# RtrMmmt/MPI-BiCGStab

Hardware: NVIDIA H100
Metric: BiCGStab iterations/sec (higher is better)
Workload: dtype f64

## Files before the change

include/bicgstab_b200.h:

```cpp
#ifndef BICGSTAB_B200_H
#define BICGSTAB_B200_H

#include <stddef.h>
#include <stdint.h>

#ifdef __cplusplus
extern "C" {
#endif

#ifndef MATRIX_H

typedef char MM_typecode[4];

typedef struct {
    double       *val;
    unsigned int *col;
    unsigned int *ptr;
    unsigned int  nz, rows, cols;
} CSR_Matrix;

typedef struct {
    unsigned int nz, rows, cols;
    MM_typecode  code;
    int         *recvcounts;
// ... 118 lines not shown
int bicg_spmv(bicg_matrix *m, const double *x_loc, double *y_loc);

int bicg_spmv_time(bicg_matrix *m, int reps, double *ms, double *bytes);

int bicg_profile_solve(bicg_matrix *m, int method, int iters, int krr, int nrr, double class_ms[3], int class_launches[3]);

int bicg_debug_vec_phase(bicg_matrix *m, int phase, const double coef[3], double *vecs, double dots[8]);
int bicg_debug_spmv_epi(bicg_matrix *m, int epi, double *vecs, double dots[8]);
int bicg_debug_get_vec(bicg_matrix *m, int id, double *out);
int bicg_debug_get_scalars(bicg_matrix *m, double out[13]);
int bicg_debug_resident_ctas(bicg_matrix *m);
int bicg_debug_coded_ctas(bicg_matrix *m);
int bicg_debug_stream_codes(bicg_matrix *m, int on);
int bicg_debug_packed_ctas(bicg_matrix *m);
int bicg_debug_stream_values(bicg_matrix *m, int on);

int bicg_last_history(double *out, int cap);
const bicg_stats *bicg_last_stats(void);

void *bicg_stream(void);
int   bicg_device(void);
void  bicg_synchronize(void);
void *bicg_host_alloc(size_t bytes);
void  bicg_host_free(void *p);

void bicg_plan_partition(int n, int world, int *counts, int *displs);
void bicg_plan_partition_nnz(const unsigned int *row_nnz, int n, int world, int *counts, int *displs);
int  bicg_plan_tiles(const unsigned int *ptr, int rows, int rows_per_tile, int cap_nnz, int *tile_row,
                     int tile_row_cap);
int  bicg_plan_cta_tiles(const unsigned int *ptr, int rows, int ctas, int rows_per_tile, const unsigned char *row_extra,
// ... 22 lines not shown
```

mpi-bicgstab_b200/_lib.py:

```python
import ctypes as C
import os

_HERE = os.path.dirname(os.path.abspath(__file__))
LIB_PATH = os.path.join(_HERE, "libbicgstab_b200.so")


class CSR_Matrix(C.Structure):
    _fields_ = [("val", C.POINTER(C.c_double)), ("col", C.POINTER(C.c_uint)), ("ptr", C.POINTER(C.c_uint)),
                ("nz", C.c_uint), ("rows", C.c_uint), ("cols", C.c_uint)]


class INFO_Matrix(C.Structure):
    _fields_ = [("nz", C.c_uint), ("rows", C.c_uint), ("cols", C.c_uint), ("code", C.c_char * 4),
                ("recvcounts", C.POINTER(C.c_int)), ("displs", C.POINTER(C.c_int))]


class bicg_stats(C.Structure):
    _fields_ = [("iters", C.c_int), ("converged", C.c_int), ("final_res", C.c_double), ("loop_ms", C.c_double),
                ("h2d_ms", C.c_double), ("d2h_ms", C.c_double), ("upload_ms", C.c_double),
                ("h2d_bytes", C.c_uint64), ("d2h_bytes", C.c_uint64), ("kernel_launches", C.c_int),
                ("spmv_lanes", C.c_int), ("spmv_kind", C.c_int)]


class bicg_result(C.Structure):
# ... 54 lines not shown
    "bicg_matrix_shift_history": (C.c_int, [C.c_void_p, _P(C.c_double), C.c_int]),
    "bicg_shift_residuals": (C.c_int, [C.c_void_p, C.c_void_p, C.c_void_p, C.c_void_p, C.c_int, C.c_int, _P(C.c_double)]),
    "bicg_last_shift_error": (C.c_int, [_P(C.c_double), C.c_int]),
    "bicg_spmv": (C.c_int, [C.c_void_p, C.c_void_p, C.c_void_p]),
    "bicg_spmv_time": (C.c_int, [C.c_void_p, C.c_int, _P(C.c_double), _P(C.c_double)]),
    "bicg_profile_solve": (C.c_int, [C.c_void_p, C.c_int, C.c_int, C.c_int, C.c_int, _P(C.c_double), _P(C.c_int)]),
    "bicg_debug_vec_phase": (C.c_int, [C.c_void_p, C.c_int, _P(C.c_double), C.c_void_p, _P(C.c_double)]),
    "bicg_debug_spmv_epi": (C.c_int, [C.c_void_p, C.c_int, C.c_void_p, _P(C.c_double)]),
    "bicg_debug_get_vec": (C.c_int, [C.c_void_p, C.c_int, C.c_void_p]),
    "bicg_debug_get_scalars": (C.c_int, [C.c_void_p, _P(C.c_double)]),
    "bicg_debug_resident_ctas": (C.c_int, [C.c_void_p]),
    "bicg_debug_coded_ctas": (C.c_int, [C.c_void_p]),
    "bicg_debug_stream_codes": (C.c_int, [C.c_void_p, C.c_int]),
    "bicg_debug_packed_ctas": (C.c_int, [C.c_void_p]),
    "bicg_debug_stream_values": (C.c_int, [C.c_void_p, C.c_int]),
    "bicg_last_history": (C.c_int, [_P(C.c_double), C.c_int]),
    "bicg_last_stats": (_P(bicg_stats), []),
    "bicg_stream": (C.c_void_p, []),
    "bicg_device": (C.c_int, []),
    "bicg_synchronize": (None, []),
    "bicg_host_alloc": (C.c_void_p, [C.c_size_t]),
    "bicg_host_free": (None, [C.c_void_p]),
    "bicg_plan_partition": (None, [C.c_int, C.c_int, _P(C.c_int), _P(C.c_int)]),
    "bicg_plan_partition_nnz": (None, [_P(C.c_uint), C.c_int, C.c_int, _P(C.c_int), _P(C.c_int)]),
    "bicg_plan_tiles": (C.c_int, [_P(C.c_uint), C.c_int, C.c_int, C.c_int, _P(C.c_int), C.c_int]),
    "bicg_plan_cta_tiles": (C.c_int, [_P(C.c_uint), C.c_int, C.c_int, C.c_int, C.c_void_p, C.c_int, _P(C.c_int), C.c_int,
                                      _P(C.c_int), _P(C.c_uint)]),
    "bicg_plan_cta_tiles_capped": (C.c_int, [_P(C.c_uint), C.c_int, C.c_int, C.c_int, C.c_int, _P(C.c_int), _P(C.c_uint), _P(C.c_int),
                                             C.c_int, _P(C.c_int), _P(C.c_uint)]),
    "bicg_plan_halo_runs": (C.c_int, [_P(CSR_Matrix), _P(INFO_Matrix), C.c_int, C.c_int, C.c_int, _P(C.c_int), C.c_int]),
# ... 26 lines not shown
```

mpi-bicgstab_b200/api.py:

```python
import ctypes as C

import numpy as np

from ._lib import ALLGATHER_FN, CSR_Matrix, INFO_Matrix, bicg_result, bicg_shift_result, bicg_stats, lib

METHODS = {"bicgstab": 0, "ca_bicgstab": 1, "pipe_bicgstab": 2, "pipe_bicgstab_rr": 3}
SHIFTED_METHODS = {"shifted_lopbicg_switching": 0, "shifted_lopbicgstab": 1, "shifted_pipe_lopbicgstab": 2}
SHIFTED_SOLVE_EX = dict(SHIFTED_METHODS, shifted_lopbicg=3)
GEN_KINDS = {"stencil15": 0, "laplace5": 1, "random": 2, "convdiff": 3}


def _dptr(a):
    return a.ctypes.data_as(C.c_void_p)


class MatrixBlock:

    def __init__(self, world):
        self.diag = CSR_Matrix()
        self.offd = CSR_Matrix()
        self.info = INFO_Matrix()
        self._recvcounts = (C.c_int * world)()
        self._displs = (C.c_int * world)()
        self.info.recvcounts = C.cast(self._recvcounts, C.POINTER(C.c_int))
# ... 430 lines not shown
    def resident_ctas(self):
        return int(lib.bicg_debug_resident_ctas(self.h))

    def coded_ctas(self):
        return int(lib.bicg_debug_coded_ctas(self.h))

    def stream_codes(self, on):
        return bool(lib.bicg_debug_stream_codes(self.h, 1 if on else 0))

    def packed_ctas(self):
        return int(lib.bicg_debug_packed_ctas(self.h))

    def stream_values(self, on):
        return bool(lib.bicg_debug_stream_values(self.h, 1 if on else 0))

    def spmv_time(self, reps=20):
        ms, by = C.c_double(), C.c_double()
        lib.bicg_spmv_time(self.h, reps, C.byref(ms), C.byref(by))
        return ms.value, by.value

    def profile(self, method, iters, krr=0, nrr=0):
        ms = (C.c_double * 3)()
        cnt = (C.c_int * 3)()
        rc = lib.bicg_profile_solve(self.h, METHODS[method], iters, int(krr), int(nrr), ms, cnt)
        if rc != 0:
            raise RuntimeError("bicg_profile_solve failed")
        return list(ms), list(cnt)

    def destroy(self):
        if self.h:
# ... 47 lines not shown
```

mpi-bicgstab_b200/csrc/engine.hpp:

```cpp
#pragma once
#include "bicgstab_b200.h"
#include "dev.cuh"
#include "plan.hpp"
#include "spmv.cuh"
#include "vec.cuh"
#include "mega.cuh"

#include <cstdio>
#include <cstdlib>
#include <functional>
#include <initializer_list>
#include <map>
#include <string>
#include <vector>

namespace bicg {

[[noreturn]] void fatal(const char *fmt, ...);
#define BICG_CUDA(call)                                                                              \
    do {                                                                                             \
        cudaError_t e_ = (call);                                                                     \
        if (e_ != cudaSuccess)                                                                       \
            ::bicg::fatal("bicgstab_b200: CUDA error %s at %s:%d: %s", cudaGetErrorName(e_), __FILE__, \
                          __LINE__, cudaGetErrorString(e_));                                          \
// ... 87 lines not shown
void load_config_from_env(Config &c);
int  set_option(Config &c, const char *key, const char *value);


struct SpmvPlan {
    int kind = 0, lanes = 1, threads = 256, stages = 3, cap = 0, grid = 0, ctas_per_sm = 1;
    size_t smem = 0;
    int ntiles = 0;
    int *d_tile_row = nullptr;
    unsigned *d_tile_nz = nullptr;
    double ms = 0.0;
};

struct MegaPlan {
    bool ok = false;
    int threads = 512, lanes = 1, stages = 2, cap = 0, grid = 0;
    size_t smem = 0;
    size_t res_smem = 0;
    int ntiles = 0;
    int *d_tile_row = nullptr;
    unsigned *d_tile_nz = nullptr;
    int *d_cta_tile = nullptr;
    int4 *d_cta_dep = nullptr;
    unsigned short *d_col16 = nullptr;
    bool stream_codes = true;
    ValTable *d_vtab = nullptr;
    unsigned char *d_vhi = nullptr;
    unsigned short *d_vmid = nullptr;
    unsigned *d_vlo = nullptr;
    bool stream_values = true;
    int *d_tile_flag = nullptr;
// ... 155 lines not shown
```

mpi-bicgstab_b200/csrc/matrix.cu:

```cuda
#include "engine.hpp"

#include <algorithm>
#include <climits>
#include <cmath>
#include <cstdarg>
#include <cstring>
#include <ctime>
#include <thread>

namespace bicg {

void fatal(const char *fmt, ...)
{
    va_list ap;
    va_start(ap, fmt);
    vfprintf(stderr, fmt, ap);
    va_end(ap);
    fputc('\n', stderr);
    exit(1);
}

namespace {

enum class Parse { Int, Double, Spmv };
// ... 442 lines not shown
    if (m->n_loc < 1) return;
    const int G = std::min(c.sm_count, MEGA_MAX_CTAS);
    const long long SMEM_MAX = 222 * 1024;
    const int lanes = c.cfg.mega_lanes > 0 ? c.cfg.mega_lanes : mega_lanes_for(m->mean_row);
    if (lanes != 1 && c.cfg.mega != 2 && c.cfg.mega_lanes == 0) return;
    for (int threads : {512, 256}) {
        if (c.cfg.mega_threads && c.cfg.mega_threads != threads) continue;
        if (!mega_has_variant(threads, lanes)) continue;
        const int rpt = threads / lanes;
        std::vector<int> tile_row, cta_tile, tile_flag;
        std::vector<unsigned> tile_nz;
        const int cap_limit = (int)(((SMEM_MAX / 2 - (long long)(rpt + 8) * 4) / 12) / 32 * 32) - 64;
        const unsigned max_tile_nnz = plan_cta_tiles(h_ptr, m->n_loc, G, rpt, row_extra.empty() ? nullptr : row_extra.data(),
                                                     c.cfg.boundary_weight, tile_row, cta_tile, cap_limit, &tile_nz, &tile_flag, c.cfg.row_weight);
        const int cap = round_up((long long)max_tile_nnz + 30, 32);
        const long long stage = (long long)cap * 12 + (long long)(rpt + 8) * 4;
        int stages = (int)std::min<long long>(4, SMEM_MAX / stage);
        if (stages < 2) continue;
        bool chunked = false;
        for (int f : tile_flag) chunked = chunked || f != 0;
        mp.chunked = chunked;
        mp.threads = threads; mp.lanes = lanes; mp.stages = stages; mp.cap = cap; mp.grid = G;
        mp.smem = mega_smem_bytes(cap, stages, threads, lanes);
        mp.res_smem = 0;
        if (lanes == 1 && !chunked) {
            size_t need = 0;
            for (int g = 0; g < G; ++g) {
                const int r0 = tile_row[(size_t)cta_tile[(size_t)g]], r1 = tile_row[(size_t)cta_tile[(size_t)g + 1]];
                need = std::max(need, mega_resident_bytes(h_ptr[r1] - h_ptr[r0], r1 - r0));
            }
            if (need <= (size_t)SMEM_MAX) mp.res_smem = std::max<size_t>(need, 16);
        }
        mp.ntiles = (int)tile_row.size() - 1;
        mp.cta_row.assign((size_t)G + 1, m->n_loc);
        for (int g = 0; g <= G; ++g) mp.cta_row[(size_t)g] = tile_row[(size_t)cta_tile[(size_t)g]];
        mp.d_tile_row = (decltype(mp.d_tile_row))c.dev_alloc(tile_row.size() * sizeof(int));
        mp.d_tile_nz = (decltype(mp.d_tile_nz))c.dev_alloc(tile_nz.size() * sizeof(unsigned));
        mp.d_cta_tile = (decltype(mp.d_cta_tile))c.dev_alloc(cta_tile.size() * sizeof(int));
// ... 2 lines not shown
        if (chunked) {
            mp.d_tile_flag = (int *)c.dev_alloc(tile_flag.size() * sizeof(int));
            BICG_CUDA(cudaMemcpy(mp.d_tile_flag, tile_flag.data(), tile_flag.size() * sizeof(int), cudaMemcpyHostToDevice));
        }
        BICG_CUDA(cudaMemcpy(mp.d_tile_row, tile_row.data(), tile_row.size() * sizeof(int), cudaMemcpyHostToDevice));
        BICG_CUDA(cudaMemcpy(mp.d_tile_nz, tile_nz.data(), tile_nz.size() * sizeof(unsigned), cudaMemcpyHostToDevice));
        BICG_CUDA(cudaMemcpy(mp.d_cta_tile, cta_tile.data(), cta_tile.size() * sizeof(int), cudaMemcpyHostToDevice));
        launch_mega_dep(m->d_col, m->d_ptr, mp.d_tile_row, mp.d_cta_tile, G, m->ghost_off, mp.d_cta_dep, c.stream);
        BICG_CUDA(cudaGetLastError());
        const size_t pad = 16;
        mp.d_col16 = (unsigned short *)c.dev_alloc((m->nnz + pad) * sizeof(unsigned short));
        BICG_CUDA(cudaMemsetAsync(mp.d_col16 + m->nnz, 0, pad * sizeof(unsigned short), c.stream));
        launch_mega_code(m->d_col, m->d_ptr, mp.d_tile_row, mp.d_cta_tile, G, m->ghost_off, mp.d_cta_dep, mp.d_col16, c.stream);
        BICG_CUDA(cudaGetLastError());
        mp.d_vtab = nullptr; mp.d_vhi = nullptr; mp.d_vmid = nullptr; mp.d_vlo = nullptr;
        if (m->mean_row >= PACK_MIN_MEAN_ROW) {
            mp.d_vtab = (ValTable *)c.dev_alloc((size_t)G * sizeof(ValTable));
            mp.d_vhi = (unsigned char *)c.dev_alloc(m->nnz + pad);
            mp.d_vmid = (unsigned short *)c.dev_alloc((m->nnz + pad) * sizeof(unsigned short));
            mp.d_vlo = (unsigned *)c.dev_alloc((m->nnz + pad) * sizeof(unsigned));
            BICG_CUDA(cudaMemsetAsync(mp.d_vhi + m->nnz, 0, pad, c.stream));
            BICG_CUDA(cudaMemsetAsync(mp.d_vmid + m->nnz, 0, pad * sizeof(unsigned short), c.stream));
            BICG_CUDA(cudaMemsetAsync(mp.d_vlo + m->nnz, 0, pad * sizeof(unsigned), c.stream));
            launch_mega_values(m->d_val, m->d_ptr, mp.d_tile_row, mp.d_cta_tile, G, m->ghost_off, mp.d_cta_dep, mp.d_vtab, mp.d_vhi,
                               mp.d_vmid, mp.d_vlo, c.stream);
            BICG_CUDA(cudaGetLastError());
        }
        mp.ok = true;
        if (c.cfg.verbose)
            fprintf(stderr, "[bicg mega r%d] threads=%d lanes=%d stages=%d cap=%d tiles=%d smem=%zu resident_smem=%zu\n", m->rank, threads, lanes,
                    stages, cap, mp.ntiles, mp.smem, mp.res_smem);
        return;
    }
}

__global__ void __launch_bounds__(256) merge_rows_kernel(int n_loc, const unsigned *__restrict__ dptr, const unsigned *__restrict__ optr,
                                                         const double *__restrict__ dval, const unsigned *__restrict__ dcol,
                                                         const double *__restrict__ oval, const unsigned *__restrict__ ocol,
                                                         const int *__restrict__ runs , int nruns, int ghost_off,
                                                         double *__restrict__ mval, unsigned *__restrict__ mcol)
{
    for (int i = blockIdx.x * blockDim.x + threadIdx.x; i < n_loc; i += gridDim.x * blockDim.x) {
        const unsigned d0 = dptr[i], d1 = dptr[i + 1], o0 = optr[i], o1 = optr[i + 1];
        unsigned k = d0 + o0;
        for (unsigned j = d0; j < d1; ++j, ++k) { mval[k] = dval[j]; mcol[k] = dcol[j]; }
        for (unsigned j = o0; j < o1; ++j, ++k) {
// ... 357 lines not shown
```

mpi-bicgstab_b200/csrc/mega.cu:

```cuda
#include "mega.cuh"
#include "vec_body.cuh"

namespace bicg {

namespace {

constexpr int RED_THREADS = MEGA_MAX_CTAS;
constexpr int RED_WARPS = RED_THREADS / 32;
struct StageHdr { int row0, row1; unsigned a0; int rowa; unsigned lo, hi; int flag; int pad_; };

__device__ __forceinline__ unsigned long long l2_evict_first_policy()
{
    unsigned long long pol;
    asm volatile("createpolicy.fractional.L2::evict_first.b64 %0, 1.0;" : "=l"(pol));
    return pol;
}
__device__ __forceinline__ void tma_load_1d_hint(unsigned dst_smem, const void *src, unsigned bytes, unsigned bar,
                                                 unsigned long long pol)
{
    asm volatile("cp.async.bulk.shared::cluster.global.mbarrier::complete_tx::bytes.L2::cache_hint [%0], [%1], %2, [%3], %4;"
                 ::"r"(dst_smem), "l"(src), "r"(bytes), "r"(bar), "l"(pol) : "memory");
}
__device__ __forceinline__ void poll_pause(unsigned spins)
{
// ... 83 lines not shown
}
__device__ __forceinline__ unsigned val_adj(const ValTable &t, int i)
{
    return i < t.n ? ((unsigned)t.field[i] << 20) - ((unsigned)i << 20) : 0u;
}
__device__ __forceinline__ unsigned lds_u32(unsigned p) { unsigned v; asm volatile("ld.shared.u32 %0, [%1];" : "=r"(v) : "r"(p)); return v; }
__device__ __forceinline__ unsigned lds_u16(unsigned p) { unsigned v; asm volatile("ld.shared.u16 %0, [%1];" : "=r"(v) : "r"(p)); return v; }
__device__ __forceinline__ unsigned lds_u8(unsigned p) { unsigned v; asm volatile("ld.shared.u8 %0, [%1];" : "=r"(v) : "r"(p)); return v; }
struct PackedVal {
    unsigned hm, lo, adj;
    __device__ __forceinline__ operator double() const
    {
        return __hiloint2double((int)(hm + lds_u32(adj + (hm >> 20) * 4u)), (int)lo);
    }
};
__device__ __forceinline__ PackedVal val_load(unsigned adj, unsigned st, unsigned cap, unsigned idx)
{
    const unsigned lo = lds_u32(st + idx * 4u), mid = lds_u16(st + cap * 4u + idx * 2u), hi = lds_u8(st + cap * 6u + idx);
    return PackedVal{(hi << 16) | mid, lo, adj};
}

template <int CT, int LANES>
struct Mega {
    static constexpr int RPT = CT / LANES, PROW = RPT + PROW_PAD, NCW = CT / 32, UNR = (LANES == 1) ? 16 : 8;
    static_assert(CT >= RED_THREADS, "the slot reduction uses one thread per CTA slot");

    const MegaArgs &a;
    MegaShared &sh;
    unsigned char *dyn;
    int tid, lane, my_tiles, row_lo, row_hi;
    unsigned vis;
    unsigned gen;
    unsigned red_epoch;
    unsigned posted_gen;
    unsigned long long halo_epoch;
    int dep_lo, dep_hi;
    unsigned push_slots;
    int ghost_lo, ghost_hi;
    int gs_lo, gs_hi;
    bool reads_ghost;
    bool is_reducer;
    size_t stage_bytes;
    int trace_it, trace_who;
    bool resident;
    bool coded;
    bool packed;
    ResidentPlan rp;
    const double *rs_val; const unsigned short *rs_col; const unsigned *rs_ptr;

    __device__ Mega(const MegaArgs &args, MegaShared &s) : a(args), sh(s) {}

    __device__ bool stop_now() const { return sh.sc.done != 0 || sh.sc.error != 0; }
    __device__ void fail() { sh.flags[3] = 1; }
    __device__ __forceinline__ bool timed_out(unsigned long long t0, unsigned spins) const
    {
        return (spins & 255u) == 0u && globaltimer_ns() - t0 > a.comm.timeout_ns;
    }
// ... 261 lines not shown
                }
#pragma unroll
                for (int u = 0; u < U; ++u) {
                    const double v = rs_val[min(min(j + (unsigned)u, e - 1u), last)];
                    if (j + (unsigned)u < e) acc = fma(v, xv[u], acc);
                }
                j += (unsigned)U;
            }
            row_done<EPI>(row, acc, e0, e1, e2, e3, y, dot);
        }
    }

    template <int EPI, bool CODED, bool PACKED>
    __device__ void spmv_impl(const double *x, double *y, double (&dot)[4])
    {
        const int stages = a.stages, cap = a.cap;
        const int sub = tid % LANES, row_in_tile = tid / LANES;
        const ColWindow w = rp.w;
        double carry = 0.0;
        for (int lt = 0; lt < my_tiles; ++lt, ++vis) {
            const int s = (int)(vis % (unsigned)stages);
            mbar_wait(smem_u32(&sh.full_bar[s]), (vis / (unsigned)stages) & 1u);
            const unsigned char *st = dyn + (size_t)s * stage_bytes;
            const double   *sval = reinterpret_cast<const double *>(st);
            const unsigned *scol = reinterpret_cast<const unsigned *>(sval + cap);
            const unsigned short *scode = reinterpret_cast<const unsigned short *>(scol);
            const unsigned *sptr = scol + cap;
            const unsigned sts = PACKED ? smem_u32(st) : 0u, adj = PACKED ? smem_u32(sh.vadj) : 0u;
            auto column = [&](unsigned idx) { return CODED ? col_decode(w, scode[idx]) : scol[idx]; };
            auto value = [&](unsigned idx) {
                if constexpr (PACKED) return val_load(adj, sts, (unsigned)cap, idx);
                else return sval[idx];
            };
            const StageHdr h = sh.hdr[s];
            if (h.flag != 0) {
                double part[1] = {0.0};
                for (unsigned jj = h.lo + (unsigned)tid; jj < h.hi; jj += 4u * CT) {
                    double pv[4], px[4];
#pragma unroll
                    for (int u = 0; u < 4; ++u) {
                        const unsigned idx = min(jj + (unsigned)(u * CT), h.hi - 1u);
                        pv[u] = (double)value(idx); px[u] = ld_coherent(x + column(idx));
                    }
#pragma unroll
                    for (int u = 0; u < 4; ++u)
                        if (jj + (unsigned)(u * CT) < h.hi) part[0] = fma(pv[u], px[u], part[0]);
// ... 278 lines not shown
            spmv<EPI_NONE>(a.v.w, a.v.t, d4);
            complete<5>(FIN_CAPIPE_END, true);
            if (stop_now()) break;
        }
    }
};

template <int CT, int LANES>
__global__ void __launch_bounds__(CT + 32, 1) bicg_mega_kernel(const __grid_constant__ MegaArgs a)
{
    using M = Mega<CT, LANES>;
    extern __shared__ __align__(128) unsigned char dyn_smem[];
    __shared__ __align__(16) MegaShared sh;

    const int tid = threadIdx.x;
    const int stages = a.stages, cap = a.cap;
    if (tid == 0) {
        for (int s = 0; s < stages; ++s) {
            mbar_init(smem_u32(&sh.full_bar[s]), 1u);
            mbar_init(smem_u32(&sh.empty_bar[s]), (unsigned)M::NCW);
        }
        sh.flags[0] = sh.flags[1] = sh.flags[2] = sh.flags[3] = 0;
        mbar_fence_init();
    }
    __syncthreads();

    const int t0 = a.cta_tile[blockIdx.x], t1 = a.cta_tile[blockIdx.x + 1];
    const int my_tiles = t1 - t0;
    const size_t stage_bytes = (size_t)cap * 12 + (size_t)M::PROW * 4;

    if (tid >= CT) {
        const ResidentPlan rp = tid == CT ? resident_plan(a, t0, t1, LANES) : ResidentPlan{};
        if (tid == CT && my_tiles > 0 && !rp.on) {
            volatile int *flags = sh.flags;
            const unsigned long long pol = l2_evict_first_policy();
            const bool coded = streams_codes(a, rp, my_tiles);
            const bool packed = streams_values(a, coded);
            const unsigned al = packed ? 15u : (coded ? 7u : 3u), cbytes = coded ? 2u : 4u, vbytes = packed ? 7u : 8u;
            const void *cols = coded ? (const void *)a.col16 : (const void *)a.col;
            unsigned v = 0;
            bool stop = false;
            for (;; ++v) {
                const int s = (int)(v % (unsigned)stages);
                if (v >= (unsigned)stages) {
                    const unsigned par = (v / (unsigned)stages - 1u) & 1u;
                    while (!mbar_try_wait(smem_u32(&sh.empty_bar[s]), par)) {
                        if (flags[1]) { stop = true; break; }
                    }
                }
                if (stop || flags[1]) break;
                const int t = t0 + (int)(v % (unsigned)my_tiles);
                const int row0 = a.tile_row[t], row1 = a.tile_row[t + 1];
                const unsigned p0 = a.tile_nz[t], p1 = a.tile_nz[t + 1];
                const auto [a0, cnt, rowa, cntp] = tile_window(row0, row1, p0, p1, al);
                unsigned char *st = dyn_smem + (size_t)s * stage_bytes;
                double   *sval = reinterpret_cast<double *>(st);
                unsigned *scol = reinterpret_cast<unsigned *>(sval + cap);
                unsigned *sptr = scol + cap;
                sh.hdr[s] = StageHdr{row0, row1, a0, rowa, p0 - a0, p1 - a0, a.tile_flag ? a.tile_flag[t] : 0, 0};
                const unsigned bar = smem_u32(&sh.full_bar[s]);
                mbar_arrive_expect_tx(bar, cnt * (vbytes + cbytes) + (unsigned)cntp * 4u);
                if (cnt) {
                    const void *csrc = (const char *)cols + (size_t)a0 * cbytes;
                    if (packed) {
                        tma_load_1d_hint(smem_u32(st), a.vlo + a0, cnt * 4u, bar, pol);
                        tma_load_1d_hint(smem_u32(st + (size_t)cap * 4u), a.vmid + a0, cnt * 2u, bar, pol);
                        tma_load_1d_hint(smem_u32(st + (size_t)cap * 6u), a.vhi + a0, cnt, bar, pol);
                    } else {
                        tma_load_1d_hint(smem_u32(sval), a.val + a0, cnt * 8u, bar, pol);
                    }
                    tma_load_1d_hint(smem_u32(scol), csrc, cnt * cbytes, bar, pol);
                }
                tma_load_1d(smem_u32(sptr), a.ptr + rowa, (unsigned)cntp * 4u, bar);
            }
            const unsigned consumed = (unsigned)flags[2];
            for (unsigned w = consumed; w < v; ++w)
                mbar_wait(smem_u32(&sh.full_bar[w % (unsigned)stages]), (w / (unsigned)stages) & 1u);
        }
    } else {
        M m(a, sh);
        m.dyn = dyn_smem; m.tid = tid; m.lane = tid & 31; m.my_tiles = my_tiles; m.vis = 0u; m.stage_bytes = stage_bytes;
        m.row_lo = a.tile_row[t0]; m.row_hi = a.tile_row[t1];
        m.trace_it = 0;
        m.trace_who = blockIdx.x == 0 ? 0 : (blockIdx.x == gridDim.x / 2 ? 1 : -1);
        m.gen = a.sync->st.gen; m.red_epoch = a.sync->st.red_epoch; m.halo_epoch = a.sync->st.halo_epoch;
        m.posted_gen = m.gen;
        if (tid == 0) sh.sc = *a.sc;

        const int4 dep = a.cta_dep[blockIdx.x];
        const int G = (int)gridDim.x;
        auto cta_of_row = [&](int r) {
            int lo = 0, hi = G;
            while (lo < hi) { const int mid = (lo + hi) >> 1; if (a.tile_row[a.cta_tile[mid]] <= r) lo = mid + 1; else hi = mid; }
            return lo - 1;
        };
        m.dep_lo = 1; m.dep_hi = 0;
// ... 25 lines not shown
        if (m.resident) {
            const size_t nnzp = ((size_t)m.rp.nnz + 7u) & ~(size_t)7u;
            double *sv = reinterpret_cast<double *>(dyn_smem);
            unsigned short *sc16 = reinterpret_cast<unsigned short *>(sv + nnzp);
            unsigned *sp = reinterpret_cast<unsigned *>(sc16 + nnzp);
            for (unsigned i = (unsigned)tid; i < m.rp.nnz; i += (unsigned)CT) {
                sv[i] = a.val[m.rp.nz_lo + i];
                sc16[i] = a.col16[m.rp.nz_lo + i];
            }
            for (int r = tid; r <= m.rp.rows; r += CT) sp[r] = a.ptr[m.rp.row_lo + r] - m.rp.nz_lo;
            m.rs_val = sv; m.rs_col = sc16; m.rs_ptr = sp;
            if (tid == 0) atomicAdd(&a.sync->st.resident_ctas, 1);
        }
        if (m.coded && tid == 0) atomicAdd(&a.sync->st.coded_ctas, 1);
        if (m.packed && tid == 0) atomicAdd(&a.sync->st.packed_ctas, 1);
        nbar(1, CT);
        if (a.comm.world > 1 && (m.reads_ghost || m.gs_hi > m.gs_lo)) {
            if (tid < 32 && !halo_wait_epoch(a.comm, sh.sc.halo_epoch) && tid == 0) { sh.sc.error = 1; sh.sc.done = 1; }
            if (tid < 32) fence_sys();
            nbar(1, CT);
        }
        if (!m.stop_now()) {
            if (a.method == 0) { if (a.comm.world > 1) m.run_bicgstab_multi(); else m.run_bicgstab(); }
            else if (a.method == 1) m.run_ca();
            else m.run_pipe(a.method == 3);
        }
        nbar(1, CT);
        if (tid == 0) {
            sh.flags[2] = (int)m.vis; __threadfence_block(); sh.flags[1] = 1;
            if (blockIdx.x == 0) {
// ... 30 lines not shown
                                                        const int *__restrict__ tile_row, const int *__restrict__ cta_tile,
                                                        int ghost_off, const int4 *__restrict__ dep, unsigned short *__restrict__ col16)
{
    const ColWindow w = col_window(dep[blockIdx.x], ghost_off);
    if (!w.ok) return;
    const int r0 = tile_row[cta_tile[blockIdx.x]], r1 = tile_row[cta_tile[blockIdx.x + 1]];
    if (r1 <= r0) return;
    const unsigned e0 = ptr[r0], e1 = ptr[r1];
    for (unsigned j = e0 + threadIdx.x; j < e1; j += blockDim.x) col16[j] = col_encode(w, ghost_off, col[j]);
}

__global__ void __launch_bounds__(256) mega_value_kernel(const double *__restrict__ val, const unsigned *__restrict__ ptr,
                                                         const int *__restrict__ tile_row, const int *__restrict__ cta_tile,
                                                         int ghost_off, const int4 *__restrict__ dep, ValTable *__restrict__ vtab,
                                                         unsigned char *__restrict__ vhi, unsigned short *__restrict__ vmid,
                                                         unsigned *__restrict__ vlo)
{
    constexpr int W = 4096 / 32;
    __shared__ unsigned seen[W];
    __shared__ int below[W];
    __shared__ int total;
    for (int i = threadIdx.x; i < W; i += blockDim.x) seen[i] = 0u;
    __syncthreads();
    const int r0 = tile_row[cta_tile[blockIdx.x]], r1 = tile_row[cta_tile[blockIdx.x + 1]];
    const unsigned e0 = r1 > r0 ? ptr[r0] : 0u, e1 = r1 > r0 ? ptr[r1] : 0u;
    for (unsigned j = e0 + threadIdx.x; j < e1; j += blockDim.x) {
        const unsigned f = (unsigned)((unsigned long long)__double_as_longlong(val[j]) >> 52), b = 1u << (f & 31u);
        if (!(seen[f >> 5] & b)) atomicOr(&seen[f >> 5], b);
    }
    __syncthreads();
    if (threadIdx.x == 0) {
        int n = 0;
        for (int i = 0; i < W; ++i) { below[i] = n; n += __popc(seen[i]); }
        total = n;
        ValTable t;
        t.n = n <= VAL_TABLE_MAX ? n : 0;
        for (int k = 0; k < VAL_TABLE_MAX; ++k) t.field[k] = 0;
        int k = 0;
        for (int i = 0; i < W && t.n > 0; ++i)
            for (unsigned b = seen[i]; b; b &= b - 1u) t.field[k++] = (unsigned short)(i * 32 + __ffs((int)b) - 1);
        vtab[blockIdx.x] = t;
    }
    __syncthreads();
    if (total == 0 || total > VAL_TABLE_MAX || !col_window(dep[blockIdx.x], ghost_off).ok) return;
    for (unsigned j = e0 + threadIdx.x; j < e1; j += blockDim.x) {
        const unsigned long long bits = (unsigned long long)__double_as_longlong(val[j]);
        const unsigned f = (unsigned)(bits >> 52);
        const unsigned idx = (unsigned)below[f >> 5] + __popc(seen[f >> 5] & ((1u << (f & 31u)) - 1u));
        vhi[j] = (unsigned char)((idx << 4) | ((unsigned)(bits >> 48) & 15u));
        vmid[j] = (unsigned short)(bits >> 32);
        vlo[j] = (unsigned)bits;
    }
}

template <int CT, int LANES>
cudaError_t launch(const MegaArgs &a, int grid, size_t smem, cudaStream_t st)
{
    void *params[1] = {(void *)&a};
    return cudaLaunchCooperativeKernel((const void *)bicg_mega_kernel<CT, LANES>, dim3(grid), dim3(CT + 32), params, smem, st);
}
template <int CT, int LANES>
cudaError_t set_attr()
{
    cudaFuncAttributes fa;
    cudaError_t e = cudaFuncGetAttributes(&fa, bicg_mega_kernel<CT, LANES>);
    if (e != cudaSuccess) return e;
    return cudaFuncSetAttribute(bicg_mega_kernel<CT, LANES>, cudaFuncAttributeMaxDynamicSharedMemorySize,
                                227 * 1024 - (int)fa.sharedSizeBytes);
}

}

size_t mega_smem_bytes(int cap, int stages, int threads, int lanes)
{
    return (size_t)stages * ((size_t)cap * 12u + (size_t)(threads / lanes + PROW_PAD) * 4u);
}

bool mega_has_variant(int threads, int lanes)
{
    if (threads == 256) return lanes == 1;
    return threads == 512 && (lanes == 1 || lanes == 4 || lanes == 8 || lanes == 32);
}

int mega_setup_attributes()
{
    cudaError_t e;
    if ((e = set_attr<256, 1>()) != cudaSuccess) return (int)e;
    if ((e = set_attr<512, 1>()) != cudaSuccess) return (int)e;
    if ((e = set_attr<512, 4>()) != cudaSuccess) return (int)e;
    if ((e = set_attr<512, 8>()) != cudaSuccess) return (int)e;
// ... 16 lines not shown

void launch_mega_dep(const unsigned *col, const unsigned *ptr, const int *tile_row, const int *cta_tile, int grid,
                     int ghost_off, int4 *dep, cudaStream_t st)
{
    mega_dep_kernel<<<grid, 256, 0, st>>>(col, ptr, tile_row, cta_tile, ghost_off, dep);
}

void launch_mega_code(const unsigned *col, const unsigned *ptr, const int *tile_row, const int *cta_tile, int grid,
                      int ghost_off, const int4 *dep, unsigned short *col16, cudaStream_t st)
{
    mega_code_kernel<<<grid, 256, 0, st>>>(col, ptr, tile_row, cta_tile, ghost_off, dep, col16);
}

void launch_mega_values(const double *val, const unsigned *ptr, const int *tile_row, const int *cta_tile, int grid,
                        int ghost_off, const int4 *dep, ValTable *vtab, unsigned char *vhi, unsigned short *vmid,
                        unsigned *vlo, cudaStream_t st)
{
    mega_value_kernel<<<grid, 256, 0, st>>>(val, ptr, tile_row, cta_tile, ghost_off, dep, vtab, vhi, vmid, vlo);
}

}
```

mpi-bicgstab_b200/csrc/mega.cuh:

```cuda
#pragma once
#include "dev.cuh"
#include "vec.cuh"

namespace bicg {

constexpr int MEGA_MAX_CTAS   = 160;
constexpr int MEGA_RING       = 8;
constexpr int MEGA_SLOT_WORDS = 16;

struct alignas(128) MegaSlot { unsigned long long w[MEGA_SLOT_WORDS]; };

struct alignas(128) MegaState {
    unsigned gen;
    unsigned red_epoch;
    unsigned long long halo_epoch;
    int plan_ok[MAX_RANKS];
    int resident_ctas;
    int coded_ctas;
    int packed_ctas;
};

struct MegaSync {
    MegaState st;
    MegaSlot  slot[MEGA_RING][MEGA_MAX_CTAS];
    MegaSlot  mail[2][MAX_RANKS];
};

struct PushPlan {
    int npeers;
    int peer[MAX_RANKS - 1];
    const PushRun *runs[MAX_RANKS - 1];
    int nruns[MAX_RANKS - 1];
    unsigned long long *ll_dst[MAX_RANKS - 1];
    long long ll_stride[MAX_RANKS - 1];
};

enum LLRegion : int { LL_S0 = 0, LL_S1, LL_R, LL_P, LL_Z, LL_X, LL_W, LL_REGIONS };

constexpr int VAL_TABLE_MAX = 16;
struct ValTable { int n; unsigned short field[VAL_TABLE_MAX]; };

constexpr int MEGA_TRACE_ITERS = 256, MEGA_TRACE_SLOTS = 16;

struct MegaArgs {
    Scalars *sc;
    double  *hist;
    CommDev  comm;
    MegaSync *sync;
    MegaSlot *peer_mail[MAX_RANKS];
    int n_ghost;
    const int4 *cta_dep;
    const double   *val;
    const unsigned *col;
    const unsigned short *col16;
    const ValTable *vtab;
    const unsigned char  *vhi;
    const unsigned short *vmid;
    const unsigned       *vlo;
    const unsigned *ptr;
    const int      *tile_row;
    const unsigned *tile_nz;
    const int      *cta_tile;
    const int      *tile_flag;
    int cap, stages;
    int ghost_off;
    int resident;
    int stream_codes;
    int stream_values;
    int smem_bytes;
    double *vec_base; long long vstride;
    VecPtrs v;
    PushPlan push;
    const unsigned long long *ll;
    long long ll_stride;
    int method;
    int krr, nrr;
    unsigned long long *snap;
    int snap_iter;
    unsigned long long *trace;
};

int    launch_mega(int threads, int lanes, int grid, size_t smem, const MegaArgs &a, cudaStream_t st);
int    mega_setup_attributes();
bool   mega_has_variant(int threads, int lanes);
size_t mega_smem_bytes(int cap, int stages, int threads, int lanes);
__host__ __device__ inline size_t mega_resident_bytes(unsigned nnz, int rows)
{
    const size_t nnzp = ((size_t)nnz + 7u) & ~(size_t)7u;
    return nnzp * 10u + ((size_t)rows + 1u) * 4u;
}
void   launch_mega_dep(const unsigned *col, const unsigned *ptr, const int *tile_row, const int *cta_tile, int grid,
                       int ghost_off, int4 *dep, cudaStream_t st);
void   launch_mega_code(const unsigned *col, const unsigned *ptr, const int *tile_row, const int *cta_tile, int grid,
                        int ghost_off, const int4 *dep, unsigned short *col16, cudaStream_t st);
void   launch_mega_values(const double *val, const unsigned *ptr, const int *tile_row, const int *cta_tile, int grid,
                          int ghost_off, const int4 *dep, ValTable *vtab, unsigned char *vhi, unsigned short *vmid,
                          unsigned *vlo, cudaStream_t st);

}
```

mpi-bicgstab_b200/csrc/solve.cu:

```cuda
#include "engine.hpp"
#include "vec_body.cuh"

#include <algorithm>
#include <cmath>
#include <cstring>

namespace bicg {

namespace {

__global__ void reset_state_kernel(Scalars *s, double tol, int max_iter)
{
    s->rTr = s->rTr_old = s->rTs = s->rTy = s->yTy = s->rTw = s->wTw = s->rTz = 0.0;
    s->dot_r = s->dot_zero = 0.0;
    s->alpha = s->beta = s->omega = 0.0;
    s->tol2 = tol * tol;
    for (int k = 0; k < MAX_DOTS; ++k) s->pend[k] = 0.0;
    s->k = 0; s->max_iter = max_iter; s->done = 0; s->converged = 0; s->error = 0; s->ticket = 0u;
}

__global__ void fill_kernel(double *p, int n, double v)
{
    for (int i = blockIdx.x * blockDim.x + threadIdx.x; i < n; i += gridDim.x * blockDim.x) p[i] = v;
}
// ... 203 lines not shown
struct Seq : PhaseLauncher {
    using PhaseLauncher::PhaseLauncher;

    bool mega(int method, int krr, int nrr)
    {
        MegaArgs a{};
        a.sc = m->d_sc; a.hist = m->d_hist; a.comm = m->comm; a.sync = m->d_msync;
        for (int p = 0; p < MAX_RANKS; ++p) a.peer_mail[p] = &m->peer_msync[p]->mail[0][0];
        a.n_ghost = m->n_ghost; a.cta_dep = m->mega.d_cta_dep;
        a.val = m->d_val; a.col = m->d_col; a.col16 = m->mega.d_col16; a.ptr = m->d_ptr;
        a.stream_codes = m->mega.stream_codes ? 1 : 0;
        a.vtab = m->mega.d_vtab; a.vhi = m->mega.d_vhi; a.vmid = m->mega.d_vmid; a.vlo = m->mega.d_vlo;
        a.stream_values = m->mega.stream_values ? 1 : 0;
        a.tile_row = m->mega.d_tile_row; a.tile_nz = m->mega.d_tile_nz; a.cta_tile = m->mega.d_cta_tile;
        a.tile_flag = m->mega.d_tile_flag;
        a.cap = m->mega.cap; a.stages = m->mega.stages;
        a.ghost_off = m->ghost_off;
        size_t smem = m->mega.smem;
        a.resident = (c.cfg.resident && m->mega.res_smem) ? 1 : 0;
        if (a.resident) smem = std::max(smem, m->mega.res_smem);
        a.smem_bytes = (int)smem;
        a.vec_base = m->vec_base; a.vstride = m->vstride;
        a.v = ptrs();
        a.push.npeers = m->world > 1 ? m->npush : 0;
        for (int s = 0; s < a.push.npeers; ++s) {
            const int d = m->push_peer[s];
            a.push.peer[s] = d;
            a.push.runs[s] = m->d_push_runs[s];
            a.push.nruns[s] = m->push_nruns[s];
            a.push.ll_dst[s] = m->peer_ll[d];
            a.push.ll_stride[s] = m->peer_ll_stride[d];
        }
        a.ll = m->d_ll; a.ll_stride = m->ll_stride;
        a.method = method; a.krr = krr; a.nrr = nrr;
        a.trace = m->d_trace;
        a.snap = m->d_trace ? m->d_trace + (size_t)2 * MEGA_TRACE_ITERS * MEGA_TRACE_SLOTS : nullptr;
        a.snap_iter = 50;
        BICG_CUDA(cudaMemsetAsync(&m->d_msync->st.resident_ctas, 0, sizeof(int), stream));
        BICG_CUDA(cudaMemsetAsync(&m->d_msync->st.coded_ctas, 0, sizeof(int), stream));
        BICG_CUDA(cudaMemsetAsync(&m->d_msync->st.packed_ctas, 0, sizeof(int), stream));
        int rc = launch_mega(m->mega.threads, m->mega.lanes, m->mega.grid, smem, a, stream);
        if (rc) {
            (void)cudaGetLastError();
            if (m->world > 1) fatal("bicgstab_b200: rank %d could not launch the persistent kernel: %s", m->rank,
                                    cudaGetErrorString((cudaError_t)rc));
            if (c.cfg.verbose) fprintf(stderr, "[bicg] persistent kernel not launched (%s); using the per-phase kernels\n",
                                       cudaGetErrorString((cudaError_t)rc));
            m->mega.ok = false;
            return false;
        }
        ++launches; ++c.launches;
        return true;
    }

    void bicgstab_init()
// ... 547 lines not shown
    return was;
}

extern "C" int bicg_debug_packed_ctas(bicg_matrix *m)
{
    using namespace bicg;
    Context &c = ctx();
    c.ensure();
    wait_handle(m);
    int n = 0;
    BICG_CUDA(cudaMemcpyAsync(&n, &m->d_msync->st.packed_ctas, sizeof(int), cudaMemcpyDeviceToHost, c.stream));
    BICG_CUDA(cudaStreamSynchronize(c.stream));
    return n;
}

extern "C" int bicg_debug_stream_values(bicg_matrix *m, int on)
{
    const int was = m->mega.stream_values ? 1 : 0;
    m->mega.stream_values = on != 0;
    return was;
}

extern "C" int bicg_profile_solve(bicg_matrix *m, int method, int iters, int krr, int nrr, double class_ms[3], int class_launches[3])
{
    using namespace bicg;
    Context &c = ctx();
    c.ensure();
    Config saved = c.cfg;
    c.cfg.tol = 0.0; c.cfg.max_iter = iters; c.cfg.quiet = 1;
    if (iters + 2 > m->hist_cap) { c.cfg = saved; return -1; }
// ... 16 lines not shown
```

Baseline: 3752.

## Size TMA staging ring per stream format so compact tiles get more stages

Replaces the fixed stage count and fixed 12-byte-per-entry stage layout with a per-format layout (packed 9, coded 10, col32 12 bytes per entry). The producer and consumers now derive the number of ring stages at runtime from the shared-memory budget and the format each CTA streams. The goal is deeper prefetch for compact formats, or a smaller shared-memory footprint when every CTA packs values. It adds a setup-time count of packing CTAs with a host sync, plus a debug counter for the stages actually used; the larger shared allocation could lower occupancy or change residency.

```diff
diff --git a/include/bicgstab_b200.h b/include/bicgstab_b200.h
--- a/include/bicgstab_b200.h
+++ b/include/bicgstab_b200.h
@@ -156,6 +156,7 @@
 int bicg_debug_stream_codes(bicg_matrix *m, int on);
 int bicg_debug_packed_ctas(bicg_matrix *m);
 int bicg_debug_stream_values(bicg_matrix *m, int on);
+int bicg_debug_ring_stages(bicg_matrix *m);
 
 int bicg_last_history(double *out, int cap);
 const bicg_stats *bicg_last_stats(void);
diff --git a/mpi-bicgstab_b200/_lib.py b/mpi-bicgstab_b200/_lib.py
--- a/mpi-bicgstab_b200/_lib.py
+++ b/mpi-bicgstab_b200/_lib.py
@@ -92,6 +92,7 @@
     "bicg_debug_stream_codes": (C.c_int, [C.c_void_p, C.c_int]),
     "bicg_debug_packed_ctas": (C.c_int, [C.c_void_p]),
     "bicg_debug_stream_values": (C.c_int, [C.c_void_p, C.c_int]),
+    "bicg_debug_ring_stages": (C.c_int, [C.c_void_p]),
     "bicg_last_history": (C.c_int, [_P(C.c_double), C.c_int]),
     "bicg_last_stats": (_P(bicg_stats), []),
     "bicg_stream": (C.c_void_p, []),
diff --git a/mpi-bicgstab_b200/api.py b/mpi-bicgstab_b200/api.py
--- a/mpi-bicgstab_b200/api.py
+++ b/mpi-bicgstab_b200/api.py
@@ -468,6 +468,9 @@
     def stream_values(self, on):
         return bool(lib.bicg_debug_stream_values(self.h, 1 if on else 0))
 
+    def ring_stages(self):
+        return int(lib.bicg_debug_ring_stages(self.h))
+
     def spmv_time(self, reps=20):
         ms, by = C.c_double(), C.c_double()
         lib.bicg_spmv_time(self.h, reps, C.byref(ms), C.byref(by))
diff --git a/mpi-bicgstab_b200/csrc/engine.hpp b/mpi-bicgstab_b200/csrc/engine.hpp
--- a/mpi-bicgstab_b200/csrc/engine.hpp
+++ b/mpi-bicgstab_b200/csrc/engine.hpp
@@ -125,7 +125,7 @@
 
 struct MegaPlan {
     bool ok = false;
-    int threads = 512, lanes = 1, stages = 2, cap = 0, grid = 0;
+    int threads = 512, lanes = 1, cap = 0, grid = 0;
     size_t smem = 0;
     size_t res_smem = 0;
     int ntiles = 0;
diff --git a/mpi-bicgstab_b200/csrc/matrix.cu b/mpi-bicgstab_b200/csrc/matrix.cu
--- a/mpi-bicgstab_b200/csrc/matrix.cu
+++ b/mpi-bicgstab_b200/csrc/matrix.cu
@@ -480,14 +480,11 @@
         const unsigned max_tile_nnz = plan_cta_tiles(h_ptr, m->n_loc, G, rpt, row_extra.empty() ? nullptr : row_extra.data(),
                                                      c.cfg.boundary_weight, tile_row, cta_tile, cap_limit, &tile_nz, &tile_flag, c.cfg.row_weight);
         const int cap = round_up((long long)max_tile_nnz + 30, 32);
-        const long long stage = (long long)cap * 12 + (long long)(rpt + 8) * 4;
-        int stages = (int)std::min<long long>(4, SMEM_MAX / stage);
-        if (stages < 2) continue;
+        if (ring_stages(SMEM_MAX, stage_layout(FMT_COL32, cap, rpt + PROW_PAD).bytes) < 2) continue;
         bool chunked = false;
         for (int f : tile_flag) chunked = chunked || f != 0;
         mp.chunked = chunked;
-        mp.threads = threads; mp.lanes = lanes; mp.stages = stages; mp.cap = cap; mp.grid = G;
-        mp.smem = mega_smem_bytes(cap, stages, threads, lanes);
+        mp.threads = threads; mp.lanes = lanes; mp.cap = cap; mp.grid = G;
         mp.res_smem = 0;
         if (lanes == 1 && !chunked) {
             size_t need = 0;
@@ -520,7 +517,10 @@
         launch_mega_code(m->d_col, m->d_ptr, mp.d_tile_row, mp.d_cta_tile, G, m->ghost_off, mp.d_cta_dep, mp.d_col16, c.stream);
         BICG_CUDA(cudaGetLastError());
         mp.d_vtab = nullptr; mp.d_vhi = nullptr; mp.d_vmid = nullptr; mp.d_vlo = nullptr;
+        int packing = 0;
         if (m->mean_row >= PACK_MIN_MEAN_ROW) {
+            int *d_packing = (int *)c.dev_alloc(sizeof(int));
+            BICG_CUDA(cudaMemsetAsync(d_packing, 0, sizeof(int), c.stream));
             mp.d_vtab = (ValTable *)c.dev_alloc((size_t)G * sizeof(ValTable));
             mp.d_vhi = (unsigned char *)c.dev_alloc(m->nnz + pad);
             mp.d_vmid = (unsigned short *)c.dev_alloc((m->nnz + pad) * sizeof(unsigned short));
@@ -529,13 +529,20 @@
             BICG_CUDA(cudaMemsetAsync(mp.d_vmid + m->nnz, 0, pad * sizeof(unsigned short), c.stream));
             BICG_CUDA(cudaMemsetAsync(mp.d_vlo + m->nnz, 0, pad * sizeof(unsigned), c.stream));
             launch_mega_values(m->d_val, m->d_ptr, mp.d_tile_row, mp.d_cta_tile, G, m->ghost_off, mp.d_cta_dep, mp.d_vtab, mp.d_vhi,
-                               mp.d_vmid, mp.d_vlo, c.stream);
+                               mp.d_vmid, mp.d_vlo, d_packing, c.stream);
             BICG_CUDA(cudaGetLastError());
-        }
+            BICG_CUDA(cudaMemcpyAsync(&packing, d_packing, sizeof(int), cudaMemcpyDeviceToHost, c.stream));
+            BICG_CUDA(cudaStreamSynchronize(c.stream));
+            c.dev_free(d_packing);
+        }
+        mp.smem = mega_smem_bytes(cap, threads, lanes, packing == G, SMEM_MAX);
+        int stages[3];
+        for (int fmt = FMT_PACKED; fmt <= FMT_COL32; ++fmt) stages[fmt] = ring_stages(mp.smem, stage_layout(fmt, cap, rpt + PROW_PAD).bytes);
         mp.ok = true;
         if (c.cfg.verbose)
-            fprintf(stderr, "[bicg mega r%d] threads=%d lanes=%d stages=%d cap=%d tiles=%d smem=%zu resident_smem=%zu\n", m->rank, threads, lanes,
-                    stages, cap, mp.ntiles, mp.smem, mp.res_smem);
+            fprintf(stderr, "[bicg mega r%d] threads=%d lanes=%d stages(9/10/12 B per entry)=%d/%d/%d cap=%d tiles=%d smem=%zu "
+                    "resident_smem=%zu\n", m->rank, threads, lanes, packing ? stages[FMT_PACKED] : 0, stages[FMT_CODED], stages[FMT_COL32],
+                    cap, mp.ntiles, mp.smem, mp.res_smem);
         return;
     }
 }
diff --git a/mpi-bicgstab_b200/csrc/mega.cu b/mpi-bicgstab_b200/csrc/mega.cu
--- a/mpi-bicgstab_b200/csrc/mega.cu
+++ b/mpi-bicgstab_b200/csrc/mega.cu
@@ -121,10 +121,14 @@
         return __hiloint2double((int)(hm + lds_u32(adj + (hm >> 20) * 4u)), (int)lo);
     }
 };
-__device__ __forceinline__ PackedVal val_load(unsigned adj, unsigned st, unsigned cap, unsigned idx)
-{
-    const unsigned lo = lds_u32(st + idx * 4u), mid = lds_u16(st + cap * 4u + idx * 2u), hi = lds_u8(st + cap * 6u + idx);
+__device__ __forceinline__ PackedVal val_load(unsigned adj, unsigned plo, unsigned pmid, unsigned phi, unsigned idx)
+{
+    const unsigned lo = lds_u32(plo + idx * 4u), mid = lds_u16(pmid + idx * 2u), hi = lds_u8(phi + idx);
     return PackedVal{(hi << 16) | mid, lo, adj};
+}
+__device__ __forceinline__ int stage_format(bool coded, bool packed)
+{
+    return packed ? FMT_PACKED : (coded ? FMT_CODED : FMT_COL32);
 }
 
 template <int CT, int LANES>
@@ -147,7 +151,6 @@
     int gs_lo, gs_hi;
     bool reads_ghost;
     bool is_reducer;
-    size_t stage_bytes;
     int trace_it, trace_who;
     bool resident;
     bool coded;
@@ -439,22 +442,23 @@
     template <int EPI, bool CODED, bool PACKED>
     __device__ void spmv_impl(const double *x, double *y, double (&dot)[4])
     {
-        const int stages = a.stages, cap = a.cap;
         const int sub = tid % LANES, row_in_tile = tid / LANES;
         const ColWindow w = rp.w;
+        const StageLayout lay = stage_layout(stage_format(CODED, PACKED), a.cap, PROW);
+        const int stages = ring_stages((size_t)a.smem_bytes, lay.bytes);
         double carry = 0.0;
         for (int lt = 0; lt < my_tiles; ++lt, ++vis) {
             const int s = (int)(vis % (unsigned)stages);
             mbar_wait(smem_u32(&sh.full_bar[s]), (vis / (unsigned)stages) & 1u);
-            const unsigned char *st = dyn + (size_t)s * stage_bytes;
+            const unsigned char *st = dyn + (size_t)s * lay.bytes;
             const double   *sval = reinterpret_cast<const double *>(st);
-            const unsigned *scol = reinterpret_cast<const unsigned *>(sval + cap);
+            const unsigned *scol = reinterpret_cast<const unsigned *>(st + lay.col);
+            const unsigned *sptr = reinterpret_cast<const unsigned *>(st + lay.ptr);
+            const unsigned sts = PACKED ? smem_u32(st) : 0u, adj = PACKED ? smem_u32(sh.vadj) : 0u;
             const unsigned short *scode = reinterpret_cast<const unsigned short *>(scol);
-            const unsigned *sptr = scol + cap;
-            const unsigned sts = PACKED ? smem_u32(st) : 0u, adj = PACKED ? smem_u32(sh.vadj) : 0u;
             auto column = [&](unsigned idx) { return CODED ? col_decode(w, scode[idx]) : scol[idx]; };
             auto value = [&](unsigned idx) {
-                if constexpr (PACKED) return val_load(adj, sts, (unsigned)cap, idx);
+                if constexpr (PACKED) return val_load(adj, sts, sts + lay.mid, sts + lay.hi, idx);
                 else return sval[idx];
             };
             const StageHdr h = sh.hdr[s];
@@ -763,9 +767,8 @@
     __shared__ __align__(16) MegaShared sh;
 
     const int tid = threadIdx.x;
-    const int stages = a.stages, cap = a.cap;
     if (tid == 0) {
-        for (int s = 0; s < stages; ++s) {
+        for (int s = 0; s < MEGA_MAX_STAGES; ++s) {
             mbar_init(smem_u32(&sh.full_bar[s]), 1u);
             mbar_init(smem_u32(&sh.empty_bar[s]), (unsigned)M::NCW);
         }
@@ -776,7 +779,6 @@
 
     const int t0 = a.cta_tile[blockIdx.x], t1 = a.cta_tile[blockIdx.x + 1];
     const int my_tiles = t1 - t0;
-    const size_t stage_bytes = (size_t)cap * 12 + (size_t)M::PROW * 4;
 
     if (tid >= CT) {
         const ResidentPlan rp = tid == CT ? resident_plan(a, t0, t1, LANES) : ResidentPlan{};
@@ -785,6 +787,8 @@
             const unsigned long long pol = l2_evict_first_policy();
             const bool coded = streams_codes(a, rp, my_tiles);
             const bool packed = streams_values(a, coded);
+            const StageLayout lay = stage_layout(stage_format(coded, packed), a.cap, M::PROW);
+            const int stages = ring_stages((size_t)a.smem_bytes, lay.bytes);
             const unsigned al = packed ? 15u : (coded ? 7u : 3u), cbytes = coded ? 2u : 4u, vbytes = packed ? 7u : 8u;
             const void *cols = coded ? (const void *)a.col16 : (const void *)a.col;
             unsigned v = 0;
@@ -802,10 +806,7 @@
                 const int row0 = a.tile_row[t], row1 = a.tile_row[t + 1];
                 const unsigned p0 = a.tile_nz[t], p1 = a.tile_nz[t + 1];
                 const auto [a0, cnt, rowa, cntp] = tile_window(row0, row1, p0, p1, al);
-                unsigned char *st = dyn_smem + (size_t)s * stage_bytes;
-                double   *sval = reinterpret_cast<double *>(st);
-                unsigned *scol = reinterpret_cast<unsigned *>(sval + cap);
-                unsigned *sptr = scol + cap;
+                unsigned char *st = dyn_smem + (size_t)s * lay.bytes;
                 sh.hdr[s] = StageHdr{row0, row1, a0, rowa, p0 - a0, p1 - a0, a.tile_flag ? a.tile_flag[t] : 0, 0};
                 const unsigned bar = smem_u32(&sh.full_bar[s]);
                 mbar_arrive_expect_tx(bar, cnt * (vbytes + cbytes) + (unsigned)cntp * 4u);
@@ -813,14 +814,14 @@
                     const void *csrc = (const char *)cols + (size_t)a0 * cbytes;
                     if (packed) {
                         tma_load_1d_hint(smem_u32(st), a.vlo + a0, cnt * 4u, bar, pol);
-                        tma_load_1d_hint(smem_u32(st + (size_t)cap * 4u), a.vmid + a0, cnt * 2u, bar, pol);
-                        tma_load_1d_hint(smem_u32(st + (size_t)cap * 6u), a.vhi + a0, cnt, bar, pol);
+                        tma_load_1d_hint(smem_u32(st + lay.mid), a.vmid + a0, cnt * 2u, bar, pol);
+                        tma_load_1d_hint(smem_u32(st + lay.hi), a.vhi + a0, cnt, bar, pol);
                     } else {
-                        tma_load_1d_hint(smem_u32(sval), a.val + a0, cnt * 8u, bar, pol);
+                        tma_load_1d_hint(smem_u32(st), a.val + a0, cnt * 8u, bar, pol);
                     }
-                    tma_load_1d_hint(smem_u32(scol), csrc, cnt * cbytes, bar, pol);
+                    tma_load_1d_hint(smem_u32(st + lay.col), csrc, cnt * cbytes, bar, pol);
                 }
-                tma_load_1d(smem_u32(sptr), a.ptr + rowa, (unsigned)cntp * 4u, bar);
+                tma_load_1d(smem_u32(st + lay.ptr), a.ptr + rowa, (unsigned)cntp * 4u, bar);
             }
             const unsigned consumed = (unsigned)flags[2];
             for (unsigned w = consumed; w < v; ++w)
@@ -828,7 +829,7 @@
         }
     } else {
         M m(a, sh);
-        m.dyn = dyn_smem; m.tid = tid; m.lane = tid & 31; m.my_tiles = my_tiles; m.vis = 0u; m.stage_bytes = stage_bytes;
+        m.dyn = dyn_smem; m.tid = tid; m.lane = tid & 31; m.my_tiles = my_tiles; m.vis = 0u;
         m.row_lo = a.tile_row[t0]; m.row_hi = a.tile_row[t1];
         m.trace_it = 0;
         m.trace_who = blockIdx.x == 0 ? 0 : (blockIdx.x == gridDim.x / 2 ? 1 : -1);
@@ -884,6 +885,8 @@
         }
         if (m.coded && tid == 0) atomicAdd(&a.sync->st.coded_ctas, 1);
         if (m.packed && tid == 0) atomicAdd(&a.sync->st.packed_ctas, 1);
+        if (!m.resident && my_tiles > 0 && tid == 0)
+            atomicMax(&a.sync->st.ring_stages, ring_stages((size_t)a.smem_bytes, stage_layout(stage_format(m.coded, m.packed), a.cap, M::PROW).bytes));
         nbar(1, CT);
         if (a.comm.world > 1 && (m.reads_ghost || m.gs_hi > m.gs_lo)) {
             if (tid < 32 && !halo_wait_epoch(a.comm, sh.sc.halo_epoch) && tid == 0) { sh.sc.error = 1; sh.sc.done = 1; }
@@ -944,7 +947,7 @@
                                                          const int *__restrict__ tile_row, const int *__restrict__ cta_tile,
                                                          int ghost_off, const int4 *__restrict__ dep, ValTable *__restrict__ vtab,
                                                          unsigned char *__restrict__ vhi, unsigned short *__restrict__ vmid,
-                                                         unsigned *__restrict__ vlo)
+                                                         unsigned *__restrict__ vlo, int *packing)
 {
     constexpr int W = 4096 / 32;
     __shared__ unsigned seen[W];
@@ -973,6 +976,7 @@
     }
     __syncthreads();
     if (total == 0 || total > VAL_TABLE_MAX || !col_window(dep[blockIdx.x], ghost_off).ok) return;
+    if (threadIdx.x == 0) atomicAdd(packing, 1);
     for (unsigned j = e0 + threadIdx.x; j < e1; j += blockDim.x) {
         const unsigned long long bits = (unsigned long long)__double_as_longlong(val[j]);
         const unsigned f = (unsigned)(bits >> 52);
@@ -1001,9 +1005,11 @@
 
 }
 
-size_t mega_smem_bytes(int cap, int stages, int threads, int lanes)
-{
-    return (size_t)stages * ((size_t)cap * 12u + (size_t)(threads / lanes + PROW_PAD) * 4u);
+size_t mega_smem_bytes(int cap, int threads, int lanes, bool all_packed, size_t budget)
+{
+    const int prow = threads / lanes + PROW_PAD;
+    const unsigned wide = stage_layout(FMT_COL32, cap, prow).bytes;
+    return (size_t)ring_stages(budget, wide) * (all_packed ? stage_layout(FMT_PACKED, cap, prow).bytes : wide);
 }
 
 bool mega_has_variant(int threads, int lanes)
@@ -1050,9 +1056,9 @@
 
 void launch_mega_values(const double *val, const unsigned *ptr, const int *tile_row, const int *cta_tile, int grid,
                         int ghost_off, const int4 *dep, ValTable *vtab, unsigned char *vhi, unsigned short *vmid,
-                        unsigned *vlo, cudaStream_t st)
-{
-    mega_value_kernel<<<grid, 256, 0, st>>>(val, ptr, tile_row, cta_tile, ghost_off, dep, vtab, vhi, vmid, vlo);
-}
-
-}
+                        unsigned *vlo, int *packing, cudaStream_t st)
+{
+    mega_value_kernel<<<grid, 256, 0, st>>>(val, ptr, tile_row, cta_tile, ghost_off, dep, vtab, vhi, vmid, vlo, packing);
+}
+
+}
diff --git a/mpi-bicgstab_b200/csrc/mega.cuh b/mpi-bicgstab_b200/csrc/mega.cuh
--- a/mpi-bicgstab_b200/csrc/mega.cuh
+++ b/mpi-bicgstab_b200/csrc/mega.cuh
@@ -18,6 +18,7 @@
     int resident_ctas;
     int coded_ctas;
     int packed_ctas;
+    int ring_stages;
 };
 
 struct MegaSync {
@@ -39,6 +40,26 @@
 
 constexpr int VAL_TABLE_MAX = 16;
 struct ValTable { int n; unsigned short field[VAL_TABLE_MAX]; };
+
+enum StageFormat : int { FMT_PACKED = 0, FMT_CODED, FMT_COL32 };
+struct StageLayout { unsigned mid, hi, col, ptr, bytes; };
+__host__ __device__ inline StageLayout stage_layout(int fmt, int cap, int prow)
+{
+    const unsigned c = (unsigned)cap, per_entry = fmt == FMT_PACKED ? 9u : (fmt == FMT_CODED ? 10u : 12u);
+    StageLayout s;
+    s.mid = 4u * c;
+    s.hi = (6u * c + 127u) & ~127u;
+    s.col = fmt == FMT_PACKED ? (s.hi + c + 127u) & ~127u : 8u * c;
+    s.ptr = ((fmt == FMT_PACKED ? s.col + 2u * c : per_entry * c) + 127u) & ~127u;
+    s.bytes = (s.ptr + 4u * (unsigned)prow + 127u) & ~127u;
+    return s;
+}
+constexpr int MEGA_MAX_STAGES = 4;
+__host__ __device__ inline int ring_stages(size_t smem_bytes, unsigned stage_bytes)
+{
+    const size_t n = smem_bytes / stage_bytes;
+    return n < (size_t)MEGA_MAX_STAGES ? (int)n : MEGA_MAX_STAGES;
+}
 
 constexpr int MEGA_TRACE_ITERS = 256, MEGA_TRACE_SLOTS = 16;
 
@@ -62,7 +83,7 @@
     const unsigned *tile_nz;
     const int      *cta_tile;
     const int      *tile_flag;
-    int cap, stages;
+    int cap;
     int ghost_off;
     int resident;
     int stream_codes;
@@ -83,7 +104,7 @@
 int    launch_mega(int threads, int lanes, int grid, size_t smem, const MegaArgs &a, cudaStream_t st);
 int    mega_setup_attributes();
 bool   mega_has_variant(int threads, int lanes);
-size_t mega_smem_bytes(int cap, int stages, int threads, int lanes);
+size_t mega_smem_bytes(int cap, int threads, int lanes, bool all_packed, size_t budget);
 __host__ __device__ inline size_t mega_resident_bytes(unsigned nnz, int rows)
 {
     const size_t nnzp = ((size_t)nnz + 7u) & ~(size_t)7u;
@@ -95,6 +116,6 @@
                         int ghost_off, const int4 *dep, unsigned short *col16, cudaStream_t st);
 void   launch_mega_values(const double *val, const unsigned *ptr, const int *tile_row, const int *cta_tile, int grid,
                           int ghost_off, const int4 *dep, ValTable *vtab, unsigned char *vhi, unsigned short *vmid,
-                          unsigned *vlo, cudaStream_t st);
+                          unsigned *vlo, int *packing, cudaStream_t st);
 
 }
diff --git a/mpi-bicgstab_b200/csrc/solve.cu b/mpi-bicgstab_b200/csrc/solve.cu
--- a/mpi-bicgstab_b200/csrc/solve.cu
+++ b/mpi-bicgstab_b200/csrc/solve.cu
@@ -241,7 +241,7 @@
         a.stream_values = m->mega.stream_values ? 1 : 0;
         a.tile_row = m->mega.d_tile_row; a.tile_nz = m->mega.d_tile_nz; a.cta_tile = m->mega.d_cta_tile;
         a.tile_flag = m->mega.d_tile_flag;
-        a.cap = m->mega.cap; a.stages = m->mega.stages;
+        a.cap = m->mega.cap;
         a.ghost_off = m->ghost_off;
         size_t smem = m->mega.smem;
         a.resident = (c.cfg.resident && m->mega.res_smem) ? 1 : 0;
@@ -266,6 +266,7 @@
         BICG_CUDA(cudaMemsetAsync(&m->d_msync->st.resident_ctas, 0, sizeof(int), stream));
         BICG_CUDA(cudaMemsetAsync(&m->d_msync->st.coded_ctas, 0, sizeof(int), stream));
         BICG_CUDA(cudaMemsetAsync(&m->d_msync->st.packed_ctas, 0, sizeof(int), stream));
+        BICG_CUDA(cudaMemsetAsync(&m->d_msync->st.ring_stages, 0, sizeof(int), stream));
         int rc = launch_mega(m->mega.threads, m->mega.lanes, m->mega.grid, smem, a, stream);
         if (rc) {
             (void)cudaGetLastError();
@@ -843,6 +844,18 @@
     return n;
 }
 
+extern "C" int bicg_debug_ring_stages(bicg_matrix *m)
+{
+    using namespace bicg;
+    Context &c = ctx();
+    c.ensure();
+    wait_handle(m);
+    int n = 0;
+    BICG_CUDA(cudaMemcpyAsync(&n, &m->d_msync->st.ring_stages, sizeof(int), cudaMemcpyDeviceToHost, c.stream));
+    BICG_CUDA(cudaStreamSynchronize(c.stream));
+    return n;
+}
+
 extern "C" int bicg_debug_stream_values(bicg_matrix *m, int on)
 {
     const int was = m->mega.stream_values ? 1 : 0;
```

Measured after the change: 3846 (median of 6 runs). 1.03x the previous value.
